# alibaba/animate-anything

Measured on NVIDIA B200. Metric: denoised_frames_per_sec_16f_512x512_50ddim, higher is better.
Workload: dtype bf16

## Files before the change

animate_anything_b200/csrc/attention.cu:

```cuda
#include "common.cuh"
#include "igemm.h"
#include <stdlib.h>

namespace aab {

constexpr int FA_THREADS = 320;
constexpr int FA_KV_STAGES = 3;
constexpr int FA_TILE_BYTES = 128 * 64 * 2;
constexpr int FA_SMEM_BYTES = 2 * FA_TILE_BYTES
                              + FA_KV_STAGES * 2 * FA_TILE_BYTES
                              + 2 * 2 * FA_TILE_BYTES
                              + 1024 + 256;

__device__ __forceinline__ float fast_exp2(float x) {
  float y;
  asm("ex2.approx.ftz.f32 %0, %1;" : "=f"(y) : "f"(x));
  return y;
}

__device__ __forceinline__ float2 ffma2(float ax, float ay, float2 b, float2 c) {
  float2 d;
  asm("{\n.reg .b64 ra, rb, rc, rd;\nmov.b64 ra, {%2, %3};\nmov.b64 rb, {%4, %5};\nmov.b64 rc, {%6, %7};\n"
      "fma.rn.f32x2 rd, ra, rb, rc;\nmov.b64 {%0, %1}, rd;\n}"
      : "=f"(d.x), "=f"(d.y)
      : "f"(ax), "f"(ay), "f"(b.x), "f"(b.y), "f"(c.x), "f"(c.y));
  return d;
}
__device__ __forceinline__ float2 fadd2(float2 a, float2 b) {
  float2 d;
  asm("{\n.reg .b64 ra, rb, rd;\nmov.b64 ra, {%2, %3};\nmov.b64 rb, {%4, %5};\nadd.rn.f32x2 rd, ra, rb;\nmov.b64 {%0, %1}, rd;\n}"
      : "=f"(d.x), "=f"(d.y)
      : "f"(a.x), "f"(a.y), "f"(b.x), "f"(b.y));
  return d;
}

__device__ __forceinline__ float2 exp2_poly2(float2 t) {
  t.x = fmaxf(t.x, -126.f);
  t.y = fmaxf(t.y, -126.f);
  const float2 magic = make_float2(12582912.f, 12582912.f);
  const float2 tt = fadd2(t, magic);
  const float2 r = fadd2(tt, make_float2(-12582912.f, -12582912.f));
  const float2 f = ffma2(r.x, r.y, make_float2(-1.f, -1.f), t);
  float2 q = ffma2(f.x, f.y, make_float2(0.00956052f, 0.00956052f), make_float2(0.05591708f, 0.05591708f));
  q = ffma2(q.x, q.y, f, make_float2(0.24024981f, 0.24024981f));
  q = ffma2(q.x, q.y, f, make_float2(0.69312196f, 0.69312196f));
  q = ffma2(q.x, q.y, f, make_float2(0.99999919f, 0.99999919f));
  float2 o;
  o.x = __int_as_float(__float_as_int(q.x) + (__float_as_int(tt.x) << 23));
  o.y = __int_as_float(__float_as_int(q.y) + (__float_as_int(tt.y) << 23));
  return o;
}

struct FaParams {
  int Lq, Lk, heads, kv_batch_div;
  int q_col0, k_col0, v_col0;
  void* out;
  long ld_out;
  long out_batch_stride;
  int out_col0;
  float scale_log2;
  int is_bf16;
  int causal;
};

__global__ void __launch_bounds__(FA_THREADS, 1)
flash_attn_d64_kernel(const __grid_constant__ CUtensorMap tmQ, const __grid_constant__ CUtensorMap tmK,
                      const __grid_constant__ CUtensorMap tmV, const FaParams p) {
  pdl_trigger();
  extern __shared__ uint8_t smem_raw[];
  uint8_t* smem = reinterpret_cast<uint8_t*>((reinterpret_cast<uintptr_t>(smem_raw) + 1023) & ~uintptr_t(1023));
  uint8_t* smQ = smem;
  uint8_t* smK = smQ + 2 * FA_TILE_BYTES;
  uint8_t* smV = smK + FA_KV_STAGES * FA_TILE_BYTES;
  uint8_t* smP = smV + FA_KV_STAGES * FA_TILE_BYTES;
  uint64_t* bars = reinterpret_cast<uint64_t*>(smP + 4 * FA_TILE_BYTES);
  uint64_t* q_full = bars;
  uint64_t* kv_full = bars + 1;
  uint64_t* kv_empty = kv_full + FA_KV_STAGES;
  uint64_t* s_full = kv_empty + FA_KV_STAGES;
  uint64_t* p_ready = s_full + 2;
  uint64_t* o_full = p_ready + 2;
  uint64_t* o_free = o_full + 2;
  uint64_t* p_free = o_free + 2;
  uint32_t* tmem_slot = reinterpret_cast<uint32_t*>(p_free + 2);

  const int warp = threadIdx.x >> 5;
  const int q0 = blockIdx.x * 256;
  const int head = blockIdx.y;
  const int b = blockIdx.z;
  const int bkv = b / p.kv_batch_div;
  const int nkv = (p.Lk + 127) / 128;
  const bool bf16 = p.is_bf16 != 0;

  if (warp == 0 && elect_one()) {
    prefetch_tmap(&tmQ);
    prefetch_tmap(&tmK);
    prefetch_tmap(&tmV);
  }
  if (warp == 1) {
    if (elect_one()) {
      mbar_init(q_full, 1);
      for (int i = 0; i < FA_KV_STAGES; ++i) {
        mbar_init(&kv_full[i], 1);
        mbar_init(&kv_empty[i], 1);
      }
      for (int i = 0; i < 2; ++i) {
        mbar_init(&s_full[i], 1);
        mbar_init(&p_ready[i], 128);
        mbar_init(&o_full[i], 1);
        mbar_init(&o_free[i], 128);
        mbar_init(&p_free[i], 1);
      }
      fence_barrier_init();
    }
    __syncwarp();
    tmem_alloc(tmem_slot, 512);
    tmem_relinquish();
  }
  tc_fence_before();
  __syncthreads();
  tc_fence_after();
  const uint32_t tmem_base = *tmem_slot;
  pdl_wait();

  if (warp == 0) {
    if (elect_one()) {
      mbar_arrive_expect_tx(q_full, 2 * FA_TILE_BYTES);
      tma_load_3d(smQ, &tmQ, q_full, p.q_col0 + head * 64, q0, b);
      tma_load_3d(smQ + FA_TILE_BYTES, &tmQ, q_full, p.q_col0 + head * 64, q0 + 128, b);
      for (int j = 0; j < nkv; ++j) {
        const int s = j % FA_KV_STAGES;
        const uint32_t ph = (j / FA_KV_STAGES) & 1;
        mbar_wait(&kv_empty[s], ph ^ 1);
        mbar_arrive_expect_tx(&kv_full[s], 2 * FA_TILE_BYTES);
        tma_load_3d(smK + s * FA_TILE_BYTES, &tmK, &kv_full[s], p.k_col0 + head * 64, j * 128, bkv);
        tma_load_3d(smV + s * FA_TILE_BYTES, &tmV, &kv_full[s], p.v_col0 + head * 64, j * 128, bkv);
      }
    }
  } else if (warp == 1) {
    const uint32_t idesc_s = make_idesc_f16(bf16 ? 1 : 0, 128, 128, 0, 0);
    const uint32_t idesc_o = make_idesc_f16(bf16 ? 1 : 0, 128, 64, 0, 1);
    auto issue_s = [&](int tile, int s) {
      if (elect_one()) {
        const uint32_t qa = smem_u32(smQ + tile * FA_TILE_BYTES);
        const uint32_t ka = smem_u32(smK + s * FA_TILE_BYTES);
#pragma unroll
        for (int k = 0; k < 4; ++k)
          umma_f16_ss(tmem_base + tile * 128, make_desc_kmajor_sw128(qa + k * 32), make_desc_kmajor_sw128(ka + k * 32),
                      idesc_s, k > 0 ? 1u : 0u);
        umma_commit(&s_full[tile]);
      }
      __syncwarp();
    };
    auto issue_pv = [&](int tile, int s) {
      if (elect_one()) {
        const uint32_t pa = smem_u32(smP + tile * 2 * FA_TILE_BYTES);
        const uint32_t va = smem_u32(smV + s * FA_TILE_BYTES);
#pragma unroll
        for (int k = 0; k < 8; ++k)
          umma_f16_ss(tmem_base + 256 + tile * 64,
                      make_desc_kmajor_sw128(pa + (k >> 2) * FA_TILE_BYTES + (k & 3) * 32),
                      make_desc_mnmajor_sw128(va + k * 2048, 8192), idesc_o, k > 0 ? 1u : 0u);
        umma_commit(&o_full[tile]);
        umma_commit(&p_free[tile]);
      }
      __syncwarp();
    };
    mbar_wait(q_full, 0);
    mbar_wait(&kv_full[0], 0);
    tc_fence_after();
    issue_s(0, 0);
    issue_s(1, 0);
    for (int j = 0; j < nkv; ++j) {
      const int s = j % FA_KV_STAGES;
      const uint32_t jph = j & 1;
      const int sn = (j + 1) % FA_KV_STAGES;
      const uint32_t phn = ((j + 1) / FA_KV_STAGES) & 1;
#pragma unroll
      for (int tile = 0; tile < 2; ++tile) {
        mbar_wait(&p_ready[tile], jph);
        if (j + 1 < nkv) {
          if (tile == 0) mbar_wait(&kv_full[sn], phn);
          tc_fence_after();
          issue_s(tile, sn);
        }
        if (j > 0) mbar_wait(&o_free[tile], jph ^ 1);
        tc_fence_after();
        issue_pv(tile, s);
        if (tile == 1 && elect_one()) umma_commit(&kv_empty[s]);
        __syncwarp();
      }
    }
  } else {
    const int tile = (warp - 2) >> 2;
    const int qd = warp & 3;
    const int row = qd * 32 + lane_id();
    const uint32_t t_s = tmem_base + tile * 128 + (static_cast<uint32_t>(qd * 32) << 16);
    const uint32_t t_o = tmem_base + 256 + tile * 64 + (static_cast<uint32_t>(qd * 32) << 16);
    uint8_t* prow = smP + tile * 2 * FA_TILE_BYTES + row * 128;
    float o_acc[64];
#pragma unroll
    for (int i = 0; i < 64; ++i) o_acc[i] = 0.f;
    float m_run = -INFINITY;
    float l_run = 0.f;
    float alpha_prev = 0.f;
    for (int j = 0; j < nkv; ++j) {
      const uint32_t jph = j & 1;
      mbar_wait(&s_full[tile], jph);
      tc_fence_after();
      const int kbase = j * 128;
      int valid = p.Lk - kbase;
      if (p.causal) {
        const int vis = q0 + tile * 128 + row - kbase + 1;
        valid = vis < valid ? vis : valid;
      }
      float alpha, lsum = 0.f;
      if (valid >= 128 && !p.causal) {
        uint32_t ra[32], rb[32];
        float mxa = -INFINITY, mxb = -INFINITY, mxc = -INFINITY, mxd = -INFINITY;
        auto max32 = [&](const uint32_t* r) {
#pragma unroll
          for (int i = 0; i < 32; i += 8) {
            mxa = fmaxf(mxa, fmaxf(__uint_as_float(r[i]), __uint_as_float(r[i + 1])));
            mxb = fmaxf(mxb, fmaxf(__uint_as_float(r[i + 2]), __uint_as_float(r[i + 3])));
            mxc = fmaxf(mxc, fmaxf(__uint_as_float(r[i + 4]), __uint_as_float(r[i + 5])));
            mxd = fmaxf(mxd, fmaxf(__uint_as_float(r[i + 6]), __uint_as_float(r[i + 7])));
          }
        };
        tmem_ld_32x32(t_s, ra);
        tmem_ld_wait();
        tmem_ld_32x32(t_s + 32, rb);
        max32(ra);
        tmem_ld_wait();
        tmem_ld_32x32(t_s + 64, ra);
        max32(rb);
        tmem_ld_wait();
        tmem_ld_32x32(t_s + 96, rb);
        max32(ra);
        tmem_ld_wait();
        tmem_ld_32x32(t_s, ra);
        max32(rb);
        const float mx = fmaxf(fmaxf(mxa, mxb), fmaxf(mxc, mxd));
        const float m_new = fmaxf(m_run, mx * p.scale_log2);
        alpha = fast_exp2(m_run - m_new);
        m_run = m_new;
        if (j > 0) mbar_wait(&p_free[tile], jph ^ 1);
        const float2 sc2 = make_float2(p.scale_log2, p.scale_log2);
        const float2 nm2 = make_float2(-m_new, -m_new);
        float2 ls[4] = {make_float2(0.f, 0.f), make_float2(0.f, 0.f), make_float2(0.f, 0.f), make_float2(0.f, 0.f)};
        auto exp32 = [&](const uint32_t* r, int c) {
          uint8_t* hp = prow + (c >> 1) * FA_TILE_BYTES;
#pragma unroll
          for (int g = 0; g < 4; ++g) {
            float2 e[4];
#pragma unroll
            for (int i = 0; i < 4; ++i) {
              const float2 t = ffma2(__uint_as_float(r[g * 8 + 2 * i]), __uint_as_float(r[g * 8 + 2 * i + 1]), sc2, nm2);
              e[i] = (i == 3) ? exp2_poly2(t) : make_float2(fast_exp2(t.x), fast_exp2(t.y));
              ls[i] = fadd2(ls[i], e[i]);
            }
            uint4 u;
            u.x = pack2(e[0].x, e[0].y, bf16);
            u.y = pack2(e[1].x, e[1].y, bf16);
            u.z = pack2(e[2].x, e[2].y, bf16);
            u.w = pack2(e[3].x, e[3].y, bf16);
            const int chunk = (c & 1) * 4 + g;
            *reinterpret_cast<uint4*>(hp + ((chunk ^ (row & 7)) << 4)) = u;
          }
        };
        exp32(rb, 3);
        tmem_ld_wait();
        tmem_ld_32x32(t_s + 32, rb);
        exp32(ra, 0);
        tmem_ld_wait();
        tmem_ld_32x32(t_s + 64, ra);
        exp32(rb, 1);
        tmem_ld_wait();
        exp32(ra, 2);
        const float2 l01 = fadd2(ls[0], ls[1]), l23 = fadd2(ls[2], ls[3]);
        lsum = (l01.x + l01.y) + (l23.x + l23.y);
      } else {
        float mx = -INFINITY;
#pragma unroll 1
        for (int c = 0; c < 4; ++c) {
          uint32_t r[32];
          tmem_ld_32x32(t_s + c * 32, r);
          tmem_ld_wait();
#pragma unroll
          for (int i = 0; i < 32; ++i)
            if (c * 32 + i < valid) mx = fmaxf(mx, __uint_as_float(r[i]));
        }
        const float m_new = fmaxf(m_run, mx * p.scale_log2);
        alpha = fast_exp2(m_run - m_new);
        m_run = m_new;
        if (j > 0) mbar_wait(&p_free[tile], jph ^ 1);
#pragma unroll 1
        for (int c = 0; c < 4; ++c) {
          uint32_t r[32];
          tmem_ld_32x32(t_s + c * 32, r);
          tmem_ld_wait();
          uint8_t* hp = prow + (c >> 1) * FA_TILE_BYTES;
#pragma unroll
          for (int g = 0; g < 4; ++g) {
            float e[8];
#pragma unroll
            for (int i = 0; i < 8; ++i) {
              const float x = fast_exp2(fmaf(__uint_as_float(r[g * 8 + i]), p.scale_log2, -m_new));
              e[i] = (c * 32 + g * 8 + i < valid) ? x : 0.f;
              lsum += e[i];
            }
            uint4 u;
            u.x = pack2(e[0], e[1], bf16);
            u.y = pack2(e[2], e[3], bf16);
            u.z = pack2(e[4], e[5], bf16);
            u.w = pack2(e[6], e[7], bf16);
            const int chunk = (c & 1) * 4 + g;
            *reinterpret_cast<uint4*>(hp + ((chunk ^ (row & 7)) << 4)) = u;
          }
        }
      }
      l_run = l_run * alpha + lsum;
      tc_fence_before();
      fence_proxy_async_smem();
      mbar_arrive(&p_ready[tile]);
      if (j > 0) {
        mbar_wait(&o_full[tile], jph ^ 1);
        tc_fence_after();
#pragma unroll
        for (int c = 0; c < 2; ++c) {
          uint32_t r[32];
          tmem_ld_32x32(t_o + c * 32, r);
          tmem_ld_wait();
#pragma unroll
          for (int i = 0; i < 32; i += 2) {
            const float2 t = ffma2(o_acc[c * 32 + i], o_acc[c * 32 + i + 1], make_float2(alpha_prev, alpha_prev),
                                   make_float2(__uint_as_float(r[i]), __uint_as_float(r[i + 1])));
            o_acc[c * 32 + i] = t.x;
            o_acc[c * 32 + i + 1] = t.y;
          }
        }
        tc_fence_before();
        mbar_arrive(&o_free[tile]);
      }
      alpha_prev = alpha;
    }
    {
      mbar_wait(&o_full[tile], (nkv - 1) & 1);
      tc_fence_after();
#pragma unroll
      for (int c = 0; c < 2; ++c) {
        uint32_t r[32];
        tmem_ld_32x32(t_o + c * 32, r);
        tmem_ld_wait();
#pragma unroll
        for (int i = 0; i < 32; ++i) o_acc[c * 32 + i] = fmaf(o_acc[c * 32 + i], alpha_prev, __uint_as_float(r[i]));
      }
    }
    const int q = q0 + tile * 128 + row;
    if (q < p.Lq) {
      const float inv = 1.0f / l_run;
      uint4* op = reinterpret_cast<uint4*>(reinterpret_cast<uint8_t*>(p.out) +
                                           (static_cast<long>(b) * p.out_batch_stride + static_cast<long>(q) * p.ld_out +
                                            p.out_col0 + head * 64) * 2);
#pragma unroll
      for (int g = 0; g < 8; ++g) {
        uint4 u;
        u.x = pack2(o_acc[g * 8 + 0] * inv, o_acc[g * 8 + 1] * inv, bf16);
        u.y = pack2(o_acc[g * 8 + 2] * inv, o_acc[g * 8 + 3] * inv, bf16);
        u.z = pack2(o_acc[g * 8 + 4] * inv, o_acc[g * 8 + 5] * inv, bf16);
        u.w = pack2(o_acc[g * 8 + 6] * inv, o_acc[g * 8 + 7] * inv, bf16);
        op[g] = u;
      }
    }
  }
  tc_fence_before();
  __syncthreads();
  if (warp == 1) {
    tc_fence_after();
    tmem_dealloc(tmem_base, 512);
  }
}

constexpr int FA2_THREADS = 192;
constexpr int FA2_SMEM_BYTES = FA_TILE_BYTES + FA_KV_STAGES * 2 * FA_TILE_BYTES + 2 * FA_TILE_BYTES + 1024 + 256;
constexpr int FA2S_SMEM_BYTES = FA_TILE_BYTES + 1 * 2 * FA_TILE_BYTES + 2 * FA_TILE_BYTES + 1024 + 256;

template <bool SHORT>
__global__ void __launch_bounds__(FA2_THREADS, SHORT ? 2 : 1)
flash_attn_d64_v2_kernel(const __grid_constant__ CUtensorMap tmQ, const __grid_constant__ CUtensorMap tmK,
                         const __grid_constant__ CUtensorMap tmV, const FaParams p) {
  pdl_trigger();
  extern __shared__ uint8_t smem_raw[];
  uint8_t* smem = reinterpret_cast<uint8_t*>((reinterpret_cast<uintptr_t>(smem_raw) + 1023) & ~uintptr_t(1023));
  constexpr int KVS = SHORT ? 1 : FA_KV_STAGES;
  constexpr uint32_t TCOLS = SHORT ? 256 : 512;
  constexpr uint32_t O_COL = SHORT ? 128 : 256;
  uint8_t* smQ = smem;
  uint8_t* smK = smQ + FA_TILE_BYTES;
  uint8_t* smV = smK + KVS * FA_TILE_BYTES;
  uint8_t* smP = smV + KVS * FA_TILE_BYTES;
  uint64_t* bars = reinterpret_cast<uint64_t*>(smP + 2 * FA_TILE_BYTES);
  uint64_t* q_full = bars;
  uint64_t* kv_full = bars + 1;
  uint64_t* kv_empty = kv_full + KVS;
  uint64_t* s_full = kv_empty + KVS;
  uint64_t* s_free = s_full + 2;
  uint64_t* p_ready = s_free + 2;
  uint64_t* p_free = p_ready + 1;
  uint64_t* o_full = p_free + 1;
  uint64_t* o_free = o_full + 1;
  uint32_t* tmem_slot = reinterpret_cast<uint32_t*>(o_free + 1);

  const int warp = threadIdx.x >> 5;
  const int q0 = blockIdx.x * 128;
  const int head = blockIdx.y;
  const int b = blockIdx.z;
  const int bkv = b / p.kv_batch_div;
  const int nkv = (p.Lk + 127) / 128;
  const bool bf16 = p.is_bf16 != 0;

  if (warp == 0 && elect_one()) {
    prefetch_tmap(&tmQ);
    prefetch_tmap(&tmK);
    prefetch_tmap(&tmV);
  }
  if (warp == 1) {
    if (elect_one()) {
      mbar_init(q_full, 1);
      for (int i = 0; i < KVS; ++i) {
// ... 536 lines not shown
  if ((ldq % 8) || (ldkv % 8) || (ld_out % 8) || (out_col0 % 8)) return AAB_ERR_ARG;
  CUtensorMap tmQ, tmK, tmV;
  int box[3] = {64, 128, 1};
  {
    long dims[3] = {q_cols, lq, nb};
    long strides[3] = {1, ldq, q_batch_stride};
    int r = make_tmap_16(&tmQ, q, 3, dims, strides, box, is_bf16);
    if (r) return r;
  }
  {
    long dims[3] = {kv_cols, lk, nb_kv};
    long strides[3] = {1, ldkv, kv_batch_stride};
    int r = make_tmap_16(&tmK, kv, 3, dims, strides, box, is_bf16);
    if (r) return r;
    tmV = tmK;
  }
  static std::atomic<unsigned long long> attr_done{0};
  if (int r = ensure_dyn_smem(flash_attn_d64_kernel, FA_SMEM_BYTES, attr_done)) return r;
  FaParams p;
  p.Lq = lq;
  p.Lk = lk;
  p.heads = heads;
  p.kv_batch_div = kv_batch_div;
  p.q_col0 = q_col0;
  p.k_col0 = k_col0;
  p.v_col0 = v_col0;
  p.out = out;
  p.ld_out = ld_out;
  p.out_batch_stride = out_batch_stride;
  p.out_col0 = out_col0;
  p.scale_log2 = scale * 1.4426950408889634f;
  p.is_bf16 = is_bf16;
  p.causal = causal;
  static int use_v1 = -1;
  if (use_v1 < 0) {
    const char* e = getenv("AAB_FLASH_V2");
    use_v1 = (e && e[0] == '1') ? 0 : 1;
  }
  static int no_short = -1;
  if (no_short < 0) {
    const char* e = getenv("AAB_FLASH_NO_SHORT");
    no_short = (e && e[0] == '1') ? 1 : 0;
  }
  if (lk <= 128 && !causal && !no_short) {
    static std::atomic<unsigned long long> attr_s{0};
    if (int r = ensure_dyn_smem(flash_attn_d64_v2_kernel<true>, FA2S_SMEM_BYTES, attr_s)) return r;
    dim3 grid((lq + 127) / 128, heads, nb);
    launch_k(flash_attn_d64_v2_kernel<true>, dim3(grid), dim3(FA2_THREADS), FA2S_SMEM_BYTES, stream, tmQ, tmK, tmV, p);
    return cudaGetLastError() == cudaSuccess ? AAB_OK : AAB_ERR_CUDA;
  }
  if (use_v1 || causal) {
    dim3 grid((lq + 255) / 256, heads, nb);
    launch_k(flash_attn_d64_kernel, dim3(grid), dim3(FA_THREADS), FA_SMEM_BYTES, stream, tmQ, tmK, tmV, p);
  } else {
    static std::atomic<unsigned long long> attr2_done{0};
    if (int r = ensure_dyn_smem(flash_attn_d64_v2_kernel<false>, FA2_SMEM_BYTES, attr2_done)) return r;
    dim3 grid((lq + 127) / 128, heads, nb);
    launch_k(flash_attn_d64_v2_kernel<false>, dim3(grid), dim3(FA2_THREADS), FA2_SMEM_BYTES, stream, tmQ, tmK, tmV, p);
  }
  return cudaGetLastError() == cudaSuccess ? AAB_OK : AAB_ERR_CUDA;
}

extern "C" int aab_temporal_attn_d64(const void* qkv, long ld, int q_col0, int k_col0, int v_col0, void* out,
                                     long ld_out, int b, int t, int hw, int heads, float scale, int is_bf16,
                                     void* stream_) {
  cudaStream_t stream = reinterpret_cast<cudaStream_t>(stream_);
  if (!qkv || !out || t < 1 || t > 32 || (ld % 8) || (ld_out % 8)) return AAB_ERR_ARG;
  const long total = static_cast<long>(b) * hw * heads;
  static int use_v1 = -1;
  if (use_v1 < 0) {
    const char* e = getenv("AAB_TATTN_V1");
    use_v1 = (e && e[0] == '1') ? 1 : 0;
  }
  if (!use_v1) {
    if ((q_col0 | k_col0 | v_col0) % 8) return AAB_ERR_ARG;
    const size_t smem2 = static_cast<size_t>(4) * 2 * TA_WARP_HALVES * sizeof(uint16_t);
    static std::atomic<unsigned long long> a2t{0}, a2f{0};
    if (int r = ensure_dyn_smem(temporal_attn_d64_v2_kernel<true>, static_cast<int>(smem2), a2t)) return r;
    if (int r = ensure_dyn_smem(temporal_attn_d64_v2_kernel<false>, static_cast<int>(smem2), a2f)) return r;
    long ctas = (total + 3) / 4;
    const long cap = 2L * num_sms();
    const int grid2 = static_cast<int>(ctas < cap ? ctas : cap);
    if (is_bf16)
      launch_k(temporal_attn_d64_v2_kernel<true>, dim3(grid2), dim3(128), smem2, stream, qkv, ld, q_col0, k_col0, v_col0, out, ld_out, b, t, hw,
                                                                       heads, scale);
    else
      launch_k(temporal_attn_d64_v2_kernel<false>, dim3(grid2), dim3(128), smem2, stream, qkv, ld, q_col0, k_col0, v_col0, out, ld_out, b, t, hw,
                                                                        heads, scale);
    return cudaGetLastError() == cudaSuccess ? AAB_OK : AAB_ERR_CUDA;
  }
  const int grid = static_cast<int>((total + 3) / 4);
  const size_t smem = static_cast<size_t>(4) * TA_WARP_HALVES * sizeof(uint16_t);
// ... 12 lines not shown
```

animate_anything_b200/csrc/common.cuh:

```cuda
#pragma once
#include <cuda.h>
#include <cuda_runtime.h>
#include <cuda_fp16.h>
#include <cuda_bf16.h>
#include <stdint.h>
#include <stdio.h>
#include <string.h>
#include <stdlib.h>
#include <atomic>

#define AAB_OK 0
#define AAB_ERR_ARG 1
#define AAB_ERR_CUDA 2
#define AAB_ERR_DRIVER 3

namespace aab {

__device__ __forceinline__ uint32_t smem_u32(const void* p) {
  return static_cast<uint32_t>(__cvta_generic_to_shared(p));
}
__device__ __forceinline__ uint32_t lane_id() { return threadIdx.x & 31; }

__device__ __forceinline__ bool elect_one() {
  uint32_t pred = 0;
// ... 20 lines not shown
__device__ __forceinline__ void mbar_arrive(uint64_t* bar) {
  asm volatile("mbarrier.arrive.shared::cta.b64 _, [%0];" ::"r"(smem_u32(bar)) : "memory");
}
__device__ __forceinline__ bool mbar_try_wait(uint64_t* bar, uint32_t parity) {
  uint32_t done;
  asm volatile(
      "{\n"
      ".reg .pred p;\n"
      "mbarrier.try_wait.parity.shared::cta.b64 p, [%1], %2;\n"
      "selp.u32 %0, 1, 0, p;\n"
      "}\n"
      : "=r"(done)
      : "r"(smem_u32(bar)), "r"(parity)
      : "memory");
  return done != 0;
}
__device__ __forceinline__ bool mbar_test_wait(uint64_t* bar, uint32_t parity) {
  uint32_t done;
  asm volatile(
      "{\n"
      ".reg .pred p;\n"
      "mbarrier.test_wait.parity.shared::cta.b64 p, [%1], %2;\n"
      "selp.u32 %0, 1, 0, p;\n"
      "}\n"
      : "=r"(done)
      : "r"(smem_u32(bar)), "r"(parity)
      : "memory");
  return done != 0;
}
__device__ __forceinline__ void mbar_wait(uint64_t* bar, uint32_t parity) {
  uint32_t spins = 0;
  while (!mbar_try_wait(bar, parity)) {
    if (++spins > (1u << 24)) {
      printf("aab: mbarrier timeout block %d thread %d bar %u parity %u\n", blockIdx.x, threadIdx.x,
             smem_u32(bar), parity);
      __trap();
    }
  }
}

__device__ __forceinline__ void prefetch_tmap(const CUtensorMap* m) {
  asm volatile("prefetch.tensormap [%0];" ::"l"(reinterpret_cast<uint64_t>(m)) : "memory");
}
__device__ __forceinline__ void tma_load_5d(void* smem_dst, const CUtensorMap* m, uint64_t* bar, int c0, int c1,
                                            int c2, int c3, int c4) {
  asm volatile(
      "cp.async.bulk.tensor.5d.shared::cluster.global.tile.mbarrier::complete_tx::bytes"
      " [%0], [%1, {%3, %4, %5, %6, %7}], [%2];"
      ::"r"(smem_u32(smem_dst)), "l"(reinterpret_cast<uint64_t>(m)), "r"(smem_u32(bar)), "r"(c0), "r"(c1),
      "r"(c2), "r"(c3), "r"(c4)
      : "memory");
}
__device__ __forceinline__ void tma_load_3d(void* smem_dst, const CUtensorMap* m, uint64_t* bar, int c0, int c1,
                                            int c2) {
  asm volatile(
      "cp.async.bulk.tensor.3d.shared::cluster.global.tile.mbarrier::complete_tx::bytes"
      " [%0], [%1, {%3, %4, %5}], [%2];"
      ::"r"(smem_u32(smem_dst)), "l"(reinterpret_cast<uint64_t>(m)), "r"(smem_u32(bar)), "r"(c0), "r"(c1), "r"(c2)
      : "memory");
}
__device__ __forceinline__ void tma_prefetch_l2_5d(const CUtensorMap* m, int c0, int c1, int c2, int c3, int c4) {
  asm volatile("cp.async.bulk.prefetch.tensor.5d.L2.global.tile [%0, {%1, %2, %3, %4, %5}];"
               ::"l"(reinterpret_cast<uint64_t>(m)), "r"(c0), "r"(c1), "r"(c2), "r"(c3), "r"(c4)
               : "memory");
}
__device__ __forceinline__ void tma_store_5d(const CUtensorMap* m, const void* smem_src, int c0, int c1, int c2,
                                             int c3, int c4) {
  asm volatile(
// ... 49 lines not shown
}
__device__ __forceinline__ void tmem_relinquish_pair() {
  asm volatile("tcgen05.relinquish_alloc_permit.cta_group::2.sync.aligned;" ::: "memory");
}
__device__ __forceinline__ void tmem_dealloc_pair(uint32_t taddr, uint32_t ncols) {
  asm volatile("tcgen05.dealloc.cta_group::2.sync.aligned.b32 %0, %1;" ::"r"(taddr), "r"(ncols) : "memory");
}
__device__ __forceinline__ void umma_f16_ss_pair(uint32_t tmem_d, uint64_t desc_a, uint64_t desc_b, uint32_t idesc,
                                                 uint32_t accumulate) {
  asm volatile(
      "{\n"
      ".reg .pred p;\n"
      "setp.ne.b32 p, %4, 0;\n"
      "tcgen05.mma.cta_group::2.kind::f16 [%0], %1, %2, %3, p;\n"
      "}\n"
      ::"r"(tmem_d), "l"(desc_a), "l"(desc_b), "r"(idesc), "r"(accumulate)
      : "memory");
}
__device__ __forceinline__ void umma_commit_pair(uint64_t* bar, uint16_t cta_mask = 3) {
  asm volatile("tcgen05.commit.cta_group::2.mbarrier::arrive::one.shared::cluster.multicast::cluster.b64 [%0], %1;"
               ::"r"(smem_u32(bar)), "h"(cta_mask)
               : "memory");
}
__device__ __forceinline__ void tma_load_3d_pair_mcast(void* smem_dst, const CUtensorMap* m, uint64_t* bar, int c0, int c1, int c2,
                                                       uint16_t cta_mask) {
  asm volatile(
      "cp.async.bulk.tensor.3d.cta_group::2.shared::cluster.global.mbarrier::complete_tx::bytes.multicast::cluster"
      " [%0], [%1, {%4, %5, %6}], [%2], %3;"
      ::"r"(smem_u32(smem_dst)), "l"(reinterpret_cast<uint64_t>(m)), "r"(smem_u32(bar) & kPeerBitMask), "h"(cta_mask), "r"(c0),
      "r"(c1), "r"(c2)
      : "memory");
}

__device__ __forceinline__ void named_bar_sync(uint32_t id, uint32_t nthreads) {
  asm volatile("bar.sync %0, %1;" ::"r"(id), "r"(nthreads) : "memory");
}

__device__ __forceinline__ void tmem_alloc(uint32_t* smem_result, uint32_t ncols) {
  asm volatile("tcgen05.alloc.cta_group::1.sync.aligned.shared::cta.b32 [%0], %1;" ::"r"(smem_u32(smem_result)),
               "r"(ncols)
               : "memory");
}
__device__ __forceinline__ void tmem_relinquish() {
  asm volatile("tcgen05.relinquish_alloc_permit.cta_group::1.sync.aligned;" ::: "memory");
}
__device__ __forceinline__ void tmem_dealloc(uint32_t taddr, uint32_t ncols) {
  asm volatile("tcgen05.dealloc.cta_group::1.sync.aligned.b32 %0, %1;" ::"r"(taddr), "r"(ncols) : "memory");
}
__device__ __forceinline__ void tc_fence_before() { asm volatile("tcgen05.fence::before_thread_sync;" ::: "memory"); }
__device__ __forceinline__ void tc_fence_after() { asm volatile("tcgen05.fence::after_thread_sync;" ::: "memory"); }

__device__ __forceinline__ void umma_f16_ss(uint32_t tmem_d, uint64_t desc_a, uint64_t desc_b, uint32_t idesc,
                                            uint32_t accumulate) {
  asm volatile(
      "{\n"
      ".reg .pred p;\n"
      "setp.ne.b32 p, %4, 0;\n"
      "tcgen05.mma.cta_group::1.kind::f16 [%0], %1, %2, %3, p;\n"
      "}\n"
      ::"r"(tmem_d), "l"(desc_a), "l"(desc_b), "r"(idesc), "r"(accumulate)
      : "memory");
}
__device__ __forceinline__ void umma_commit(uint64_t* bar) {
  asm volatile("tcgen05.commit.cta_group::1.mbarrier::arrive::one.shared::cluster.b64 [%0];" ::"r"(smem_u32(bar))
               : "memory");
}
__device__ __forceinline__ void tmem_ld_wait() { asm volatile("tcgen05.wait::ld.sync.aligned;" ::: "memory"); }

__device__ __forceinline__ void tmem_ld_32x32(uint32_t taddr, uint32_t* r) {
  asm volatile(
      "tcgen05.ld.sync.aligned.32x32b.x32.b32 "
      "{%0, %1, %2, %3, %4, %5, %6, %7, %8, %9, %10, %11, %12, %13, %14, %15, "
      "%16, %17, %18, %19, %20, %21, %22, %23, %24, %25, %26, %27, %28, %29, %30, %31}, [%32];"
      : "=r"(r[0]), "=r"(r[1]), "=r"(r[2]), "=r"(r[3]), "=r"(r[4]), "=r"(r[5]), "=r"(r[6]), "=r"(r[7]), "=r"(r[8]),
        "=r"(r[9]), "=r"(r[10]), "=r"(r[11]), "=r"(r[12]), "=r"(r[13]), "=r"(r[14]), "=r"(r[15]), "=r"(r[16]),
        "=r"(r[17]), "=r"(r[18]), "=r"(r[19]), "=r"(r[20]), "=r"(r[21]), "=r"(r[22]), "=r"(r[23]), "=r"(r[24]),
        "=r"(r[25]), "=r"(r[26]), "=r"(r[27]), "=r"(r[28]), "=r"(r[29]), "=r"(r[30]), "=r"(r[31])
      : "r"(taddr)
      : "memory");
}

__device__ __forceinline__ void tmem_ld_32x16(uint32_t taddr, uint32_t* r) {
  asm volatile(
      "tcgen05.ld.sync.aligned.32x32b.x16.b32 "
      "{%0, %1, %2, %3, %4, %5, %6, %7, %8, %9, %10, %11, %12, %13, %14, %15}, [%16];"
      : "=r"(r[0]), "=r"(r[1]), "=r"(r[2]), "=r"(r[3]), "=r"(r[4]), "=r"(r[5]), "=r"(r[6]), "=r"(r[7]), "=r"(r[8]),
        "=r"(r[9]), "=r"(r[10]), "=r"(r[11]), "=r"(r[12]), "=r"(r[13]), "=r"(r[14]), "=r"(r[15])
      : "r"(taddr)
      : "memory");
}

__device__ __forceinline__ uint64_t make_desc_kmajor_sw128(uint32_t smem_addr) {
  uint64_t d = 0;
  d |= static_cast<uint64_t>((smem_addr & 0x3FFFF) >> 4);
  d |= static_cast<uint64_t>(1) << 16;
  d |= static_cast<uint64_t>(1024 >> 4) << 32;
  d |= static_cast<uint64_t>(1) << 46;
  d |= static_cast<uint64_t>(2) << 61;
  return d;
}
__device__ __forceinline__ uint64_t make_desc_mnmajor_sw128(uint32_t smem_addr, uint32_t lbo_bytes) {
  uint64_t d = 0;
  d |= static_cast<uint64_t>((smem_addr & 0x3FFFF) >> 4);
  d |= static_cast<uint64_t>((lbo_bytes >> 4) & 0x3FFF) << 16;
  d |= static_cast<uint64_t>(1024 >> 4) << 32;
  d |= static_cast<uint64_t>(1) << 46;
  d |= static_cast<uint64_t>(2) << 61;
  return d;
}

__host__ __device__ inline uint32_t make_idesc_f16(int is_bf16, int M, int N, int a_mn, int b_mn) {
  uint32_t d = 0;
  d |= 1u << 4;
  d |= static_cast<uint32_t>(is_bf16 ? 1 : 0) << 7;
  d |= static_cast<uint32_t>(is_bf16 ? 1 : 0) << 10;
  d |= static_cast<uint32_t>(a_mn ? 1 : 0) << 15;
  d |= static_cast<uint32_t>(b_mn ? 1 : 0) << 16;
  d |= static_cast<uint32_t>(N >> 3) << 17;
  d |= static_cast<uint32_t>(M >> 4) << 24;
  return d;
}

template <typename Kernel>
// ... 97 lines not shown
```

Measured before the change: 5.175.

## Restructure flash attention: P in TMEM, smem O accumulator, register reallocation

Reworks the main d64 flash attention kernel. P is now stored into tensor memory and the PV product uses the TMEM-A MMA form instead of writing P to swizzled shared memory. The running O accumulator moves from registers into shared memory, and a new s_free barrier lets the next S MMA start as soon as the S tile has been read. Control warps are moved to the end and give up registers via setmaxnreg, so the softmax warps can hold the full 128-wide row. It also removes the v2 env-selected path and merges the tail softmax logic, at the cost of extra shared-memory traffic for O and a more complex barrier protocol.

New measurement: 5.183 (median of 6 runs). No clear change (+0.2%).

```diff
diff --git a/animate_anything_b200/csrc/attention.cu b/animate_anything_b200/csrc/attention.cu
--- a/animate_anything_b200/csrc/attention.cu
+++ b/animate_anything_b200/csrc/attention.cu
@@ -4,13 +4,15 @@
 
 namespace aab {
 
-constexpr int FA_THREADS = 320;
+constexpr int FA_THREADS = 384;
+constexpr uint32_t FA_SOFTMAX_REGS = 216, FA_CONTROL_REGS = 72;
 constexpr int FA_KV_STAGES = 3;
 constexpr int FA_TILE_BYTES = 128 * 64 * 2;
 constexpr int FA_SMEM_BYTES = 2 * FA_TILE_BYTES
                               + FA_KV_STAGES * 2 * FA_TILE_BYTES
-                              + 2 * 2 * FA_TILE_BYTES
+                              + 2 * FA_TILE_BYTES * 2
                               + 1024 + 256;
+constexpr uint32_t FA_S_COL = 0, FA_P_COL = 256, FA_O_COL = 384;
 
 __device__ __forceinline__ float fast_exp2(float x) {
   float y;
@@ -63,6 +65,53 @@
   int causal;
 };
 
+__device__ __forceinline__ float fa_rowmax(const uint32_t (&r)[128]) {
+  float a = -INFINITY, b = -INFINITY, c = -INFINITY, d = -INFINITY;
+#pragma unroll
+  for (int i = 0; i < 128; i += 8) {
+    a = fmaxf(a, fmaxf(__uint_as_float(r[i]), __uint_as_float(r[i + 1])));
+    b = fmaxf(b, fmaxf(__uint_as_float(r[i + 2]), __uint_as_float(r[i + 3])));
+    c = fmaxf(c, fmaxf(__uint_as_float(r[i + 4]), __uint_as_float(r[i + 5])));
+    d = fmaxf(d, fmaxf(__uint_as_float(r[i + 6]), __uint_as_float(r[i + 7])));
+  }
+  return fmaxf(fmaxf(a, b), fmaxf(c, d));
+}
+
+template <bool TAIL>
+__device__ __forceinline__ float fa_exp_pack(const uint32_t (&r)[128], uint32_t (&pk)[64], float scale_log2, float m, int valid,
+                                             bool bf16) {
+  const float2 sc2 = make_float2(scale_log2, scale_log2);
+  const float2 nm2 = make_float2(-m, -m);
+  if (TAIL) {
+    float lsum = 0.f;
+#pragma unroll
+    for (int i = 0; i < 64; ++i) {
+      const float2 t = ffma2(__uint_as_float(r[2 * i]), __uint_as_float(r[2 * i + 1]), sc2, nm2);
+      const float ex = 2 * i < valid ? fast_exp2(t.x) : 0.f;
+      const float ey = 2 * i + 1 < valid ? fast_exp2(t.y) : 0.f;
+      lsum += ex;
+      lsum += ey;
+      pk[i] = pack2(ex, ey, bf16);
+    }
+    return lsum;
+  }
+  float2 ls[4] = {make_float2(0.f, 0.f), make_float2(0.f, 0.f), make_float2(0.f, 0.f), make_float2(0.f, 0.f)};
+#pragma unroll
+  for (int cc = 0; cc < 4; ++cc) {
+    const int c = (cc + 3) & 3;
+#pragma unroll
+    for (int q = 0; q < 16; ++q) {
+      const int i = c * 16 + q;
+      const float2 t = ffma2(__uint_as_float(r[2 * i]), __uint_as_float(r[2 * i + 1]), sc2, nm2);
+      const float2 e = (q & 3) == 3 ? exp2_poly2(t) : make_float2(fast_exp2(t.x), fast_exp2(t.y));
+      ls[q & 3] = fadd2(ls[q & 3], e);
+      pk[i] = pack2(e.x, e.y, bf16);
+    }
+  }
+  const float2 l01 = fadd2(ls[0], ls[1]), l23 = fadd2(ls[2], ls[3]);
+  return (l01.x + l01.y) + (l23.x + l23.y);
+}
+
 __global__ void __launch_bounds__(FA_THREADS, 1)
 flash_attn_d64_kernel(const __grid_constant__ CUtensorMap tmQ, const __grid_constant__ CUtensorMap tmK,
                       const __grid_constant__ CUtensorMap tmV, const FaParams p) {
@@ -72,16 +121,15 @@
   uint8_t* smQ = smem;
   uint8_t* smK = smQ + 2 * FA_TILE_BYTES;
   uint8_t* smV = smK + FA_KV_STAGES * FA_TILE_BYTES;
-  uint8_t* smP = smV + FA_KV_STAGES * FA_TILE_BYTES;
-  uint64_t* bars = reinterpret_cast<uint64_t*>(smP + 4 * FA_TILE_BYTES);
+  float* smO = reinterpret_cast<float*>(smV + FA_KV_STAGES * FA_TILE_BYTES);
+  uint64_t* bars = reinterpret_cast<uint64_t*>(smO + 2 * 128 * 64);
   uint64_t* q_full = bars;
   uint64_t* kv_full = bars + 1;
   uint64_t* kv_empty = kv_full + FA_KV_STAGES;
   uint64_t* s_full = kv_empty + FA_KV_STAGES;
-  uint64_t* p_ready = s_full + 2;
-  uint64_t* o_full = p_ready + 2;
-  uint64_t* o_free = o_full + 2;
-  uint64_t* p_free = o_free + 2;
+  uint64_t* s_free = s_full + 2;
+  uint64_t* p_ready = s_free + 2;
+  uint64_t* p_free = p_ready + 2;
   uint32_t* tmem_slot = reinterpret_cast<uint32_t*>(p_free + 2);
 
   const int warp = threadIdx.x >> 5;
@@ -92,12 +140,12 @@
   const int nkv = (p.Lk + 127) / 128;
   const bool bf16 = p.is_bf16 != 0;
 
-  if (warp == 0 && elect_one()) {
+  if (warp == 8 && elect_one()) {
     prefetch_tmap(&tmQ);
     prefetch_tmap(&tmK);
     prefetch_tmap(&tmV);
   }
-  if (warp == 1) {
+  if (warp == 9) {
     if (elect_one()) {
       mbar_init(q_full, 1);
       for (int i = 0; i < FA_KV_STAGES; ++i) {
@@ -106,9 +154,8 @@
       }
       for (int i = 0; i < 2; ++i) {
         mbar_init(&s_full[i], 1);
+        mbar_init(&s_free[i], 128);
         mbar_init(&p_ready[i], 128);
-        mbar_init(&o_full[i], 1);
-        mbar_init(&o_free[i], 128);
         mbar_init(&p_free[i], 1);
       }
       fence_barrier_init();
@@ -123,8 +170,9 @@
   const uint32_t tmem_base = *tmem_slot;
   pdl_wait();
 
-  if (warp == 0) {
-    if (elect_one()) {
+  if (warp >= 8) {
+    setmaxnreg_dec<FA_CONTROL_REGS>();
+    if (warp == 8 && elect_one()) {
       mbar_arrive_expect_tx(q_full, 2 * FA_TILE_BYTES);
       tma_load_3d(smQ, &tmQ, q_full, p.q_col0 + head * 64, q0, b);
       tma_load_3d(smQ + FA_TILE_BYTES, &tmQ, q_full, p.q_col0 + head * 64, q0 + 128, b);
@@ -136,225 +184,144 @@
         tma_load_3d(smK + s * FA_TILE_BYTES, &tmK, &kv_full[s], p.k_col0 + head * 64, j * 128, bkv);
         tma_load_3d(smV + s * FA_TILE_BYTES, &tmV, &kv_full[s], p.v_col0 + head * 64, j * 128, bkv);
       }
-    }
-  } else if (warp == 1) {
-    const uint32_t idesc_s = make_idesc_f16(bf16 ? 1 : 0, 128, 128, 0, 0);
-    const uint32_t idesc_o = make_idesc_f16(bf16 ? 1 : 0, 128, 64, 0, 1);
-    auto issue_s = [&](int tile, int s) {
-      if (elect_one()) {
-        const uint32_t qa = smem_u32(smQ + tile * FA_TILE_BYTES);
-        const uint32_t ka = smem_u32(smK + s * FA_TILE_BYTES);
-#pragma unroll
-        for (int k = 0; k < 4; ++k)
-          umma_f16_ss(tmem_base + tile * 128, make_desc_kmajor_sw128(qa + k * 32), make_desc_kmajor_sw128(ka + k * 32),
-                      idesc_s, k > 0 ? 1u : 0u);
-        umma_commit(&s_full[tile]);
-      }
-      __syncwarp();
-    };
-    auto issue_pv = [&](int tile, int s) {
-      if (elect_one()) {
-        const uint32_t pa = smem_u32(smP + tile * 2 * FA_TILE_BYTES);
-        const uint32_t va = smem_u32(smV + s * FA_TILE_BYTES);
-#pragma unroll
-        for (int k = 0; k < 8; ++k)
-          umma_f16_ss(tmem_base + 256 + tile * 64,
-                      make_desc_kmajor_sw128(pa + (k >> 2) * FA_TILE_BYTES + (k & 3) * 32),
-                      make_desc_mnmajor_sw128(va + k * 2048, 8192), idesc_o, k > 0 ? 1u : 0u);
-        umma_commit(&o_full[tile]);
-        umma_commit(&p_free[tile]);
-      }
-      __syncwarp();
-    };
-    mbar_wait(q_full, 0);
-    mbar_wait(&kv_full[0], 0);
-    tc_fence_after();
-    issue_s(0, 0);
-    issue_s(1, 0);
-    for (int j = 0; j < nkv; ++j) {
-      const int s = j % FA_KV_STAGES;
-      const uint32_t jph = j & 1;
-      const int sn = (j + 1) % FA_KV_STAGES;
-      const uint32_t phn = ((j + 1) / FA_KV_STAGES) & 1;
-#pragma unroll
-      for (int tile = 0; tile < 2; ++tile) {
-        mbar_wait(&p_ready[tile], jph);
+    } else if (warp == 9) {
+      const uint32_t idesc_s = make_idesc_f16(bf16 ? 1 : 0, 128, 128, 0, 0);
+      const uint32_t idesc_o = make_idesc_f16(bf16 ? 1 : 0, 128, 64, 0, 1);
+      auto issue_s = [&](int tile, int s) {
+        if (elect_one()) {
+          const uint32_t qa = smem_u32(smQ + tile * FA_TILE_BYTES);
+          const uint32_t ka = smem_u32(smK + s * FA_TILE_BYTES);
+#pragma unroll
+          for (int k = 0; k < 4; ++k)
+            umma_f16_ss(tmem_base + FA_S_COL + tile * 128, make_desc_kmajor_sw128(qa + k * 32),
+                        make_desc_kmajor_sw128(ka + k * 32), idesc_s, k > 0 ? 1u : 0u);
+          umma_commit(&s_full[tile]);
+        }
+        __syncwarp();
+      };
+      auto issue_pv = [&](int tile, int s) {
+        if (elect_one()) {
+          const uint32_t va = smem_u32(smV + s * FA_TILE_BYTES);
+#pragma unroll
+          for (int k = 0; k < 8; ++k)
+            umma_f16_ts(tmem_base + FA_O_COL + tile * 64, tmem_base + FA_P_COL + tile * 64 + k * 8,
+                        make_desc_mnmajor_sw128(va + k * 2048, 8192), idesc_o, k > 0 ? 1u : 0u);
+          umma_commit(&p_free[tile]);
+        }
+        __syncwarp();
+      };
+      mbar_wait(q_full, 0);
+      mbar_wait(&kv_full[0], 0);
+      tc_fence_after();
+      issue_s(0, 0);
+      issue_s(1, 0);
+      for (int j = 0; j < nkv; ++j) {
+        const int s = j % FA_KV_STAGES;
+        const uint32_t jph = j & 1;
         if (j + 1 < nkv) {
-          if (tile == 0) mbar_wait(&kv_full[sn], phn);
+          const int sn = (j + 1) % FA_KV_STAGES;
+          mbar_wait(&kv_full[sn], ((j + 1) / FA_KV_STAGES) & 1);
+#pragma unroll
+          for (int tile = 0; tile < 2; ++tile) {
+            mbar_wait(&s_free[tile], jph);
+            tc_fence_after();
+            issue_s(tile, sn);
+          }
+        }
+#pragma unroll
+        for (int tile = 0; tile < 2; ++tile) {
+          mbar_wait(&p_ready[tile], jph);
           tc_fence_after();
-          issue_s(tile, sn);
+          issue_pv(tile, s);
         }
-        if (j > 0) mbar_wait(&o_free[tile], jph ^ 1);
-        tc_fence_after();
-        issue_pv(tile, s);
-        if (tile == 1 && elect_one()) umma_commit(&kv_empty[s]);
+        if (elect_one()) umma_commit(&kv_empty[s]);
         __syncwarp();
       }
     }
   } else {
-    const int tile = (warp - 2) >> 2;
+    setmaxnreg_inc<FA_SOFTMAX_REGS>();
+    const int tile = warp >> 2;
     const int qd = warp & 3;
     const int row = qd * 32 + lane_id();
-    const uint32_t t_s = tmem_base + tile * 128 + (static_cast<uint32_t>(qd * 32) << 16);
-    const uint32_t t_o = tmem_base + 256 + tile * 64 + (static_cast<uint32_t>(qd * 32) << 16);
-    uint8_t* prow = smP + tile * 2 * FA_TILE_BYTES + row * 128;
-    float o_acc[64];
-#pragma unroll
-    for (int i = 0; i < 64; ++i) o_acc[i] = 0.f;
+    const uint32_t lane_off = static_cast<uint32_t>(qd * 32) << 16;
+    const uint32_t t_s = tmem_base + FA_S_COL + tile * 128 + lane_off;
+    const uint32_t t_p = tmem_base + FA_P_COL + tile * 64 + lane_off;
+    const uint32_t t_o = tmem_base + FA_O_COL + tile * 64 + lane_off;
+    float* o_acc = smO + (tile * 16 * 128 + row) * 4;
+#pragma unroll
+    for (int g = 0; g < 16; ++g) *reinterpret_cast<float4*>(o_acc + g * 512) = make_float4(0.f, 0.f, 0.f, 0.f);
     float m_run = -INFINITY;
     float l_run = 0.f;
     float alpha_prev = 0.f;
+    auto accumulate = [&](int half, const uint32_t (&o)[32], float alpha) {
+#pragma unroll
+      for (int g = 8 * half; g < 8 * half + 8; ++g) {
+        const float4 a = *reinterpret_cast<float4*>(o_acc + g * 512);
+        const float2 lo = ffma2(a.x, a.y, make_float2(alpha, alpha),
+                                make_float2(__uint_as_float(o[4 * g - 32 * half]), __uint_as_float(o[4 * g + 1 - 32 * half])));
+        const float2 hi = ffma2(a.z, a.w, make_float2(alpha, alpha),
+                                make_float2(__uint_as_float(o[4 * g + 2 - 32 * half]), __uint_as_float(o[4 * g + 3 - 32 * half])));
+        *reinterpret_cast<float4*>(o_acc + g * 512) = make_float4(lo.x, lo.y, hi.x, hi.y);
+      }
+    };
     for (int j = 0; j < nkv; ++j) {
       const uint32_t jph = j & 1;
       mbar_wait(&s_full[tile], jph);
       tc_fence_after();
-      const int kbase = j * 128;
-      int valid = p.Lk - kbase;
+      uint32_t r[128];
+      tmem_ld_32x32(t_s, r);
+      tmem_ld_32x32(t_s + 32, r + 32);
+      tmem_ld_32x32(t_s + 64, r + 64);
+      tmem_ld_32x32(t_s + 96, r + 96);
+      tmem_ld_wait();
+      tc_fence_before();
+      mbar_arrive(&s_free[tile]);
+      int valid = p.Lk - j * 128;
       if (p.causal) {
-        const int vis = q0 + tile * 128 + row - kbase + 1;
+        const int vis = q0 + tile * 128 + row + 1;
         valid = vis < valid ? vis : valid;
       }
-      float alpha, lsum = 0.f;
-      if (valid >= 128 && !p.causal) {
-        uint32_t ra[32], rb[32];
-        float mxa = -INFINITY, mxb = -INFINITY, mxc = -INFINITY, mxd = -INFINITY;
-        auto max32 = [&](const uint32_t* r) {
-#pragma unroll
-          for (int i = 0; i < 32; i += 8) {
-            mxa = fmaxf(mxa, fmaxf(__uint_as_float(r[i]), __uint_as_float(r[i + 1])));
-            mxb = fmaxf(mxb, fmaxf(__uint_as_float(r[i + 2]), __uint_as_float(r[i + 3])));
-            mxc = fmaxf(mxc, fmaxf(__uint_as_float(r[i + 4]), __uint_as_float(r[i + 5])));
-            mxd = fmaxf(mxd, fmaxf(__uint_as_float(r[i + 6]), __uint_as_float(r[i + 7])));
-          }
-        };
-        tmem_ld_32x32(t_s, ra);
-        tmem_ld_wait();
-        tmem_ld_32x32(t_s + 32, rb);
-        max32(ra);
-        tmem_ld_wait();
-        tmem_ld_32x32(t_s + 64, ra);
-        max32(rb);
-        tmem_ld_wait();
-        tmem_ld_32x32(t_s + 96, rb);
-        max32(ra);
-        tmem_ld_wait();
-        tmem_ld_32x32(t_s, ra);
-        max32(rb);
-        const float mx = fmaxf(fmaxf(mxa, mxb), fmaxf(mxc, mxd));
-        const float m_new = fmaxf(m_run, mx * p.scale_log2);
-        alpha = fast_exp2(m_run - m_new);
-        m_run = m_new;
-        if (j > 0) mbar_wait(&p_free[tile], jph ^ 1);
-        const float2 sc2 = make_float2(p.scale_log2, p.scale_log2);
-        const float2 nm2 = make_float2(-m_new, -m_new);
-        float2 ls[4] = {make_float2(0.f, 0.f), make_float2(0.f, 0.f), make_float2(0.f, 0.f), make_float2(0.f, 0.f)};
-        auto exp32 = [&](const uint32_t* r, int c) {
-          uint8_t* hp = prow + (c >> 1) * FA_TILE_BYTES;
-#pragma unroll
-          for (int g = 0; g < 4; ++g) {
-            float2 e[4];
-#pragma unroll
-            for (int i = 0; i < 4; ++i) {
-              const float2 t = ffma2(__uint_as_float(r[g * 8 + 2 * i]), __uint_as_float(r[g * 8 + 2 * i + 1]), sc2, nm2);
-              e[i] = (i == 3) ? exp2_poly2(t) : make_float2(fast_exp2(t.x), fast_exp2(t.y));
-              ls[i] = fadd2(ls[i], e[i]);
-            }
-            uint4 u;
-            u.x = pack2(e[0].x, e[0].y, bf16);
-            u.y = pack2(e[1].x, e[1].y, bf16);
-            u.z = pack2(e[2].x, e[2].y, bf16);
-            u.w = pack2(e[3].x, e[3].y, bf16);
-            const int chunk = (c & 1) * 4 + g;
-            *reinterpret_cast<uint4*>(hp + ((chunk ^ (row & 7)) << 4)) = u;
-          }
-        };
-        exp32(rb, 3);
-        tmem_ld_wait();
-        tmem_ld_32x32(t_s + 32, rb);
-        exp32(ra, 0);
-        tmem_ld_wait();
-        tmem_ld_32x32(t_s + 64, ra);
-        exp32(rb, 1);
-        tmem_ld_wait();
-        exp32(ra, 2);
-        const float2 l01 = fadd2(ls[0], ls[1]), l23 = fadd2(ls[2], ls[3]);
-        lsum = (l01.x + l01.y) + (l23.x + l23.y);
-      } else {
-        float mx = -INFINITY;
-#pragma unroll 1
-        for (int c = 0; c < 4; ++c) {
-          uint32_t r[32];
-          tmem_ld_32x32(t_s + c * 32, r);
+      const bool tail = p.causal || valid < 128;
+      if (tail) {
+#pragma unroll
+        for (int i = 0; i < 128; ++i)
+          if (i >= valid) r[i] = 0xff800000u;
+      }
+      const float m_new = fmaxf(m_run, fa_rowmax(r) * p.scale_log2);
+      const float alpha = fast_exp2(m_run - m_new);
+      m_run = m_new;
+      uint32_t pk[64];
+      const float lsum = tail ? fa_exp_pack<true>(r, pk, p.scale_log2, m_new, valid, bf16)
+                              : fa_exp_pack<false>(r, pk, p.scale_log2, m_new, valid, bf16);
+      l_run = l_run * alpha + lsum;
+      if (j > 0) {
+        mbar_wait(&p_free[tile], jph ^ 1);
+        tc_fence_after();
+      }
+      tmem_st_32x32(t_p, pk);
+      tmem_st_32x32(t_p + 32, pk + 32);
+      if (j > 0) {
+#pragma unroll
+        for (int h = 0; h < 2; ++h) {
+          uint32_t o[32];
+          tmem_ld_32x32(t_o + h * 32, o);
           tmem_ld_wait();
-#pragma unroll
-          for (int i = 0; i < 32; ++i)
-            if (c * 32 + i < valid) mx = fmaxf(mx, __uint_as_float(r[i]));
+          accumulate(h, o, alpha_prev);
         }
-        const float m_new = fmaxf(m_run, mx * p.scale_log2);
-        alpha = fast_exp2(m_run - m_new);
-        m_run = m_new;
-        if (j > 0) mbar_wait(&p_free[tile], jph ^ 1);
-#pragma unroll 1
-        for (int c = 0; c < 4; ++c) {
-          uint32_t r[32];
-          tmem_ld_32x32(t_s + c * 32, r);
-          tmem_ld_wait();
-          uint8_t* hp = prow + (c >> 1) * FA_TILE_BYTES;
-#pragma unroll
-          for (int g = 0; g < 4; ++g) {
-            float e[8];
-#pragma unroll
-            for (int i = 0; i < 8; ++i) {
-              const float x = fast_exp2(fmaf(__uint_as_float(r[g * 8 + i]), p.scale_log2, -m_new));
-              e[i] = (c * 32 + g * 8 + i < valid) ? x : 0.f;
-              lsum += e[i];
-            }
-            uint4 u;
-            u.x = pack2(e[0], e[1], bf16);
-            u.y = pack2(e[2], e[3], bf16);
-            u.z = pack2(e[4], e[5], bf16);
-            u.w = pack2(e[6], e[7], bf16);
-            const int chunk = (c & 1) * 4 + g;
-            *reinterpret_cast<uint4*>(hp + ((chunk ^ (row & 7)) << 4)) = u;
-          }
-        }
-      }
-      l_run = l_run * alpha + lsum;
+      }
+      tmem_st_wait();
       tc_fence_before();
-      fence_proxy_async_smem();
       mbar_arrive(&p_ready[tile]);
-      if (j > 0) {
-        mbar_wait(&o_full[tile], jph ^ 1);
-        tc_fence_after();
-#pragma unroll
-        for (int c = 0; c < 2; ++c) {
-          uint32_t r[32];
-          tmem_ld_32x32(t_o + c * 32, r);
-          tmem_ld_wait();
-#pragma unroll
-          for (int i = 0; i < 32; i += 2) {
-            const float2 t = ffma2(o_acc[c * 32 + i], o_acc[c * 32 + i + 1], make_float2(alpha_prev, alpha_prev),
-                                   make_float2(__uint_as_float(r[i]), __uint_as_float(r[i + 1])));
-            o_acc[c * 32 + i] = t.x;
-            o_acc[c * 32 + i + 1] = t.y;
-          }
-        }
-        tc_fence_before();
-        mbar_arrive(&o_free[tile]);
-      }
       alpha_prev = alpha;
     }
-    {
-      mbar_wait(&o_full[tile], (nkv - 1) & 1);
-      tc_fence_after();
-#pragma unroll
-      for (int c = 0; c < 2; ++c) {
-        uint32_t r[32];
-        tmem_ld_32x32(t_o + c * 32, r);
-        tmem_ld_wait();
-#pragma unroll
-        for (int i = 0; i < 32; ++i) o_acc[c * 32 + i] = fmaf(o_acc[c * 32 + i], alpha_prev, __uint_as_float(r[i]));
-      }
+    mbar_wait(&p_free[tile], (nkv - 1) & 1);
+    tc_fence_after();
+#pragma unroll
+    for (int h = 0; h < 2; ++h) {
+      uint32_t o[32];
+      tmem_ld_32x32(t_o + h * 32, o);
+      tmem_ld_wait();
+      accumulate(h, o, alpha_prev);
     }
     const int q = q0 + tile * 128 + row;
     if (q < p.Lq) {
@@ -365,36 +332,36 @@
 #pragma unroll
       for (int g = 0; g < 8; ++g) {
         uint4 u;
-        u.x = pack2(o_acc[g * 8 + 0] * inv, o_acc[g * 8 + 1] * inv, bf16);
-        u.y = pack2(o_acc[g * 8 + 2] * inv, o_acc[g * 8 + 3] * inv, bf16);
-        u.z = pack2(o_acc[g * 8 + 4] * inv, o_acc[g * 8 + 5] * inv, bf16);
-        u.w = pack2(o_acc[g * 8 + 6] * inv, o_acc[g * 8 + 7] * inv, bf16);
+        const float4 a = *reinterpret_cast<const float4*>(o_acc + 2 * g * 512);
+        const float4 c = *reinterpret_cast<const float4*>(o_acc + (2 * g + 1) * 512);
+        u.x = pack2(a.x * inv, a.y * inv, bf16);
+        u.y = pack2(a.z * inv, a.w * inv, bf16);
+        u.z = pack2(c.x * inv, c.y * inv, bf16);
+        u.w = pack2(c.z * inv, c.w * inv, bf16);
         op[g] = u;
       }
     }
   }
   tc_fence_before();
   __syncthreads();
-  if (warp == 1) {
+  if (warp == 9) {
     tc_fence_after();
     tmem_dealloc(tmem_base, 512);
   }
 }
 
 constexpr int FA2_THREADS = 192;
-constexpr int FA2_SMEM_BYTES = FA_TILE_BYTES + FA_KV_STAGES * 2 * FA_TILE_BYTES + 2 * FA_TILE_BYTES + 1024 + 256;
 constexpr int FA2S_SMEM_BYTES = FA_TILE_BYTES + 1 * 2 * FA_TILE_BYTES + 2 * FA_TILE_BYTES + 1024 + 256;
 
-template <bool SHORT>
-__global__ void __launch_bounds__(FA2_THREADS, SHORT ? 2 : 1)
-flash_attn_d64_v2_kernel(const __grid_constant__ CUtensorMap tmQ, const __grid_constant__ CUtensorMap tmK,
-                         const __grid_constant__ CUtensorMap tmV, const FaParams p) {
+__global__ void __launch_bounds__(FA2_THREADS, 2)
+flash_attn_d64_short_kernel(const __grid_constant__ CUtensorMap tmQ, const __grid_constant__ CUtensorMap tmK,
+                            const __grid_constant__ CUtensorMap tmV, const FaParams p) {
   pdl_trigger();
   extern __shared__ uint8_t smem_raw[];
   uint8_t* smem = reinterpret_cast<uint8_t*>((reinterpret_cast<uintptr_t>(smem_raw) + 1023) & ~uintptr_t(1023));
-  constexpr int KVS = SHORT ? 1 : FA_KV_STAGES;
-  constexpr uint32_t TCOLS = SHORT ? 256 : 512;
-  constexpr uint32_t O_COL = SHORT ? 128 : 256;
+  constexpr int KVS = 1;
+  constexpr uint32_t TCOLS = 256;
+  constexpr uint32_t O_COL = 128;
   uint8_t* smQ = smem;
   uint8_t* smK = smQ + FA_TILE_BYTES;
   uint8_t* smV = smK + KVS * FA_TILE_BYTES;
@@ -997,11 +964,6 @@
   p.scale_log2 = scale * 1.4426950408889634f;
   p.is_bf16 = is_bf16;
   p.causal = causal;
-  static int use_v1 = -1;
-  if (use_v1 < 0) {
-    const char* e = getenv("AAB_FLASH_V2");
-    use_v1 = (e && e[0] == '1') ? 0 : 1;
-  }
   static int no_short = -1;
   if (no_short < 0) {
     const char* e = getenv("AAB_FLASH_NO_SHORT");
@@ -1009,20 +971,13 @@
   }
   if (lk <= 128 && !causal && !no_short) {
     static std::atomic<unsigned long long> attr_s{0};
-    if (int r = ensure_dyn_smem(flash_attn_d64_v2_kernel<true>, FA2S_SMEM_BYTES, attr_s)) return r;
+    if (int r = ensure_dyn_smem(flash_attn_d64_short_kernel, FA2S_SMEM_BYTES, attr_s)) return r;
     dim3 grid((lq + 127) / 128, heads, nb);
-    launch_k(flash_attn_d64_v2_kernel<true>, dim3(grid), dim3(FA2_THREADS), FA2S_SMEM_BYTES, stream, tmQ, tmK, tmV, p);
+    launch_k(flash_attn_d64_short_kernel, dim3(grid), dim3(FA2_THREADS), FA2S_SMEM_BYTES, stream, tmQ, tmK, tmV, p);
     return cudaGetLastError() == cudaSuccess ? AAB_OK : AAB_ERR_CUDA;
   }
-  if (use_v1 || causal) {
-    dim3 grid((lq + 255) / 256, heads, nb);
-    launch_k(flash_attn_d64_kernel, dim3(grid), dim3(FA_THREADS), FA_SMEM_BYTES, stream, tmQ, tmK, tmV, p);
-  } else {
-    static std::atomic<unsigned long long> attr2_done{0};
-    if (int r = ensure_dyn_smem(flash_attn_d64_v2_kernel<false>, FA2_SMEM_BYTES, attr2_done)) return r;
-    dim3 grid((lq + 127) / 128, heads, nb);
-    launch_k(flash_attn_d64_v2_kernel<false>, dim3(grid), dim3(FA2_THREADS), FA2_SMEM_BYTES, stream, tmQ, tmK, tmV, p);
-  }
+  dim3 grid((lq + 255) / 256, heads, nb);
+  launch_k(flash_attn_d64_kernel, dim3(grid), dim3(FA_THREADS), FA_SMEM_BYTES, stream, tmQ, tmK, tmV, p);
   return cudaGetLastError() == cudaSuccess ? AAB_OK : AAB_ERR_CUDA;
 }
 
diff --git a/animate_anything_b200/csrc/common.cuh b/animate_anything_b200/csrc/common.cuh
--- a/animate_anything_b200/csrc/common.cuh
+++ b/animate_anything_b200/csrc/common.cuh
@@ -76,8 +76,9 @@
   uint32_t spins = 0;
   while (!mbar_try_wait(bar, parity)) {
     if (++spins > (1u << 24)) {
-      printf("aab: mbarrier timeout block %d thread %d bar %u parity %u\n", blockIdx.x, threadIdx.x,
-             smem_u32(bar), parity);
+      uint32_t cta, tid;
+      asm volatile("mov.u32 %0, %%ctaid.x;\n\tmov.u32 %1, %%tid.x;" : "=r"(cta), "=r"(tid));
+      printf("aab: mbarrier timeout block %u thread %u bar %u parity %u\n", cta, tid, smem_u32(bar), parity);
       __trap();
     }
   }
@@ -193,6 +194,11 @@
       : "memory");
 }
 
+template <uint32_t N>
+__device__ __forceinline__ void setmaxnreg_dec() { asm volatile("setmaxnreg.dec.sync.aligned.u32 %0;" ::"n"(N)); }
+template <uint32_t N>
+__device__ __forceinline__ void setmaxnreg_inc() { asm volatile("setmaxnreg.inc.sync.aligned.u32 %0;" ::"n"(N)); }
+
 __device__ __forceinline__ void named_bar_sync(uint32_t id, uint32_t nthreads) {
   asm volatile("bar.sync %0, %1;" ::"r"(id), "r"(nthreads) : "memory");
 }
@@ -220,6 +226,17 @@
       "tcgen05.mma.cta_group::1.kind::f16 [%0], %1, %2, %3, p;\n"
       "}\n"
       ::"r"(tmem_d), "l"(desc_a), "l"(desc_b), "r"(idesc), "r"(accumulate)
+      : "memory");
+}
+__device__ __forceinline__ void umma_f16_ts(uint32_t tmem_d, uint32_t tmem_a, uint64_t desc_b, uint32_t idesc,
+                                            uint32_t accumulate) {
+  asm volatile(
+      "{\n"
+      ".reg .pred p;\n"
+      "setp.ne.b32 p, %4, 0;\n"
+      "tcgen05.mma.cta_group::1.kind::f16 [%0], [%1], %2, %3, p;\n"
+      "}\n"
+      ::"r"(tmem_d), "r"(tmem_a), "l"(desc_b), "r"(idesc), "r"(accumulate)
       : "memory");
 }
 __device__ __forceinline__ void umma_commit(uint64_t* bar) {
@@ -250,6 +267,19 @@
       : "r"(taddr)
       : "memory");
 }
+
+__device__ __forceinline__ void tmem_st_32x32(uint32_t taddr, const uint32_t* r) {
+  asm volatile(
+      "tcgen05.st.sync.aligned.32x32b.x32.b32 [%0], "
+      "{%1, %2, %3, %4, %5, %6, %7, %8, %9, %10, %11, %12, %13, %14, %15, %16, "
+      "%17, %18, %19, %20, %21, %22, %23, %24, %25, %26, %27, %28, %29, %30, %31, %32};"
+      ::"r"(taddr), "r"(r[0]), "r"(r[1]), "r"(r[2]), "r"(r[3]), "r"(r[4]), "r"(r[5]), "r"(r[6]), "r"(r[7]), "r"(r[8]),
+      "r"(r[9]), "r"(r[10]), "r"(r[11]), "r"(r[12]), "r"(r[13]), "r"(r[14]), "r"(r[15]), "r"(r[16]), "r"(r[17]),
+      "r"(r[18]), "r"(r[19]), "r"(r[20]), "r"(r[21]), "r"(r[22]), "r"(r[23]), "r"(r[24]), "r"(r[25]), "r"(r[26]),
+      "r"(r[27]), "r"(r[28]), "r"(r[29]), "r"(r[30]), "r"(r[31])
+      : "memory");
+}
+__device__ __forceinline__ void tmem_st_wait() { asm volatile("tcgen05.wait::st.sync.aligned;" ::: "memory"); }
 
 __device__ __forceinline__ uint64_t make_desc_kmajor_sw128(uint32_t smem_addr) {
   uint64_t d = 0;
```
